# ku222/Attention-GAN

Measured on AMD Instinct MI355X. Metric: train images/sec at 256×256 stage-3, batch 24/GPU, 1/2/4/8 MI355X, higher is better.
Workload: dtype f32; 1 GPU; full 3-stage AttnGAN 64->128->256 train step: G + 3xD updates + word attention + DAMSM words/sentence loss + KL + 4x fused Adam (BASELINE.json configs[2]); workload_key=full3, batch_per_gpu=24, global_batch=24, gf_dim=32, df_dim=64, emb_dim=256, seq_len=10, text_encoder=bypassed (frozen; N(0,1) embeddings), parallelism=dp1, discriminator_streams=3, launch=eager, gradient_exchange=none (one rank), losses_finite=True

## Files before the change

### attention-gan_amd/csrc/conv_wino.hip

```cpp
#include "conv_common.h"

#include <cstring>
#include <type_traits>

using namespace agan;
using namespace agan::conv;

namespace {

typedef unsigned u32x4 __attribute__((ext_vector_type(4)));

__device__ __forceinline__ void lds_barrier_w() { asm volatile("s_waitcnt lgkmcnt(0)\n\ts_barrier" ::: "memory"); }

__global__ __launch_bounds__(256) void wino_weight_transform_kernel(const float* __restrict__ wk, float* __restrict__ U, int Kin, int Nld, int N) {
    const int total = Kin * Nld;
    for (int e = blockIdx.x * 256 + threadIdx.x; e < total; e += gridDim.x * 256) {
        const int n = e % Nld, c = e / Nld;
        float gk[3][3];
#pragma unroll
        for (int r = 0; r < 3; ++r)
#pragma unroll
            for (int s = 0; s < 3; ++s) gk[r][s] = n < N ? wk[(size_t)(c * 9 + r * 3 + s) * Nld + n] : 0.f;
        float t[4][3];
#pragma unroll
        for (int s = 0; s < 3; ++s) {
            t[0][s] = gk[0][s];
            t[1][s] = 0.5f * (gk[0][s] + gk[1][s] + gk[2][s]);
            t[2][s] = 0.5f * (gk[0][s] - gk[1][s] + gk[2][s]);
            t[3][s] = gk[2][s];
        }
        const int nch8 = Kin >> 3;
#pragma unroll
        for (int xi = 0; xi < 4; ++xi) {
            const float u0 = t[xi][0], u1 = 0.5f * (t[xi][0] + t[xi][1] + t[xi][2]), u2 = 0.5f * (t[xi][0] - t[xi][1] + t[xi][2]), u3 = t[xi][2];
            const float u[4] = {u0, u1, u2, u3};
#pragma unroll
            for (int nu = 0; nu < 4; ++nu) U[((size_t)((xi * 4 + nu) * nch8 + (c >> 3)) * Nld + n) * 8 + (c & 7)] = u[nu];
        }
    }
}

struct WinoTraits {
    int step, extra, origin;
    int cch;
    int planes, classes;
    int stages, nacc;
    int vfrags;
    int pieces;
    int ni32, ni64;
    int lds_cap;
    int s_u_second, s_raw_load, s_u_next, s_transform, s_raw_store;
    bool mulshift;
    bool store1_late;
};
constexpr WinoTraits wino_traits(WinoKind k) {
    WinoTraits t{};
    t.origin = -1; t.classes = 1; t.lds_cap = 160 * 1024; t.s_u_second = 0; t.s_raw_load = 1;
    switch (k) {
    case WinoKind::conv3x3:
        t.step = 2; t.extra = 2; t.cch = 8; t.planes = 16; t.stages = 16; t.nacc = 16; t.vfrags = 16; t.pieces = 4; t.ni32 = 7; t.ni64 = 11;
        t.s_u_next = 8; t.s_transform = 1; t.s_raw_store = 14;
        break;
    case WinoKind::conv3x3_half:
        t.step = 2; t.extra = 2; t.cch = 8; t.planes = 16; t.stages = 8; t.nacc = 8; t.vfrags = 16; t.pieces = 4; t.ni32 = 7;
        t.s_u_next = 4; t.s_transform = 1; t.s_raw_store = 6; t.lds_cap = 80 * 1024; t.mulshift = true;
        break;
    case WinoKind::conv4x4_s2:
        t.step = 4; t.extra = 2; t.cch = 8; t.planes = 36; t.stages = 36; t.nacc = 9; t.vfrags = 36; t.pieces = 4; t.ni32 = 21;
        t.s_u_next = 18; t.s_transform = 2; t.s_raw_store = 32; t.store1_late = true;
        break;
    case WinoKind::dgrad2x2_class:
        t.step = 2; t.extra = 1; t.cch = 16; t.planes = 36; t.classes = 4; t.stages = 18; t.nacc = 9; t.vfrags = 18; t.pieces = 2; t.ni32 = 11;
        t.s_u_next = 9; t.s_transform = 2; t.s_raw_store = 15; t.store1_late = true;
        break;
    }
    return t;
}

template <int D>
__device__ __forceinline__ void wino_input_f22(const float* src, int pcp, float* o, int pp) {
    float t[3][3];
#pragma unroll
    for (int j = 0; j < 3; ++j) {
        const float d0 = src[D * j], d1 = src[D * pcp + D * j], d2 = src[2 * D * pcp + D * j];
        t[0][j] = d0 - d1; t[1][j] = d1; t[2][j] = d2 - d1;
    }
#pragma unroll
    for (int xi = 0; xi < 3; ++xi) {
        o[(xi * 3 + 0) * pp] = t[xi][0] - t[xi][1]; o[(xi * 3 + 1) * pp] = t[xi][1]; o[(xi * 3 + 2) * pp] = t[xi][2] - t[xi][1];
    }
}

template <int NACC>
__device__ __forceinline__ void wino_output_2x2(const f32x16 (&acc)[NACC], int r, float (&y)[4]) {
    if constexpr (NACC == 16) {
        float c0[4], c1[4];
#pragma unroll
        for (int nu = 0; nu < 4; ++nu) {
            c0[nu] = acc[0 + nu][r] + acc[4 + nu][r] + acc[8 + nu][r];
            c1[nu] = acc[4 + nu][r] - acc[8 + nu][r] - acc[12 + nu][r];
        }
        y[0] = c0[0] + c0[1] + c0[2]; y[1] = c0[1] - c0[2] - c0[3];
        y[2] = c1[0] + c1[1] + c1[2]; y[3] = c1[1] - c1[2] - c1[3];
    } else {
        static_assert(NACC == 9, "F(2x2, 3x3) or F(2x2, 2x2)");
        float c0[3], c1[3];
#pragma unroll
        for (int nu = 0; nu < 3; ++nu) {
            c0[nu] = acc[nu][r] + acc[3 + nu][r];
            c1[nu] = acc[3 + nu][r] + acc[6 + nu][r];
        }
        y[0] = c0[0] + c0[1]; y[1] = c0[1] + c0[2];
        y[2] = c1[0] + c1[1]; y[3] = c1[1] + c1[2];
    }
}

template <WinoKind K, int NTG>
struct WinoGather {
    static constexpr WinoTraits T = wino_traits(K);
    static constexpr bool kHalf = K == WinoKind::conv3x3_half, kS2 = K == WinoKind::conv4x4_s2, kCls = K == WinoKind::dgrad2x2_class;
    static constexpr bool k3x3 = T.nacc != 9;
    static constexpr int NFW = kHalf ? 2 : 4 / NTG;
    static constexpr int NTL = 32 * NTG, LT = NTG == 1 ? 5 : 6;
    static constexpr int NI = NTG == 1 ? T.ni32 : T.ni64;
    static constexpr int CCH = T.cch, C8 = T.cch / 8;
    static constexpr int S = T.stages, SH = T.stages / 2, NACC = T.nacc;
    static constexpr int NPIECE = T.pieces * NTG;
    static constexpr int VBUF = T.vfrags * NTL * 8;
    static constexpr int STEP = T.step;
    static_assert(NI > 0, "this block size of the variant is not built: plan_wino must not route to it");
    static_assert(T.s_u_next == SH && T.s_transform + NPIECE <= S && T.s_raw_store < S, "slots of the chunk loop");

    const Geom& g;
    const WinoPlan& wp;
    int tid, lane, w, fw, tg, hh, l31, lh;
    int mt, nt, ks, py, px;
    int n0, txl, tyl, TX, TY, tx0, ty0, tb0, ihw, ohw, PR, PC, PCP, RAWBUF;
    float *raw, *V;
    __amdgpu_buffer_rsrc_t rx, rU;
    int nch8, c_beg, nch;
    int iy0, ix0;

    __device__ __forceinline__ WinoGather(const float* x, const float* U, const Geom& g_, const WinoPlan& wp_) : g(g_), wp(wp_) {
        extern __shared__ __attribute__((aligned(16))) unsigned char lds[];
        tid = threadIdx.x; lane = tid & 63;
        w = __builtin_amdgcn_readfirstlane(tid >> 6);
        fw = w % NFW; tg = kHalf ? 0 : w / NFW; hh = kHalf ? w / NFW : 0;
        l31 = lane & 31; lh = lane >> 5;
        ks = py = px = 0;
        {
            int F = xcd_contiguous(linear_block_id(), wp.mtiles * wp.ntiles * (kS2 ? wp.ksplit : T.classes));
            nt = F % wp.ntiles; F /= wp.ntiles;
            if constexpr (kS2) { mt = F % wp.mtiles; ks = F / wp.mtiles; }
            else if constexpr (kCls) { py = (F & 3) >> 1; px = F & 1; mt = F >> 2; }
            else mt = F;
        }
        n0 = nt * (NFW * 32);
        txl = wp.txl; tyl = wp.tyl;
        TX = 1 << txl; TY = 1 << tyl;
        const int bxi = mt % wp.blocks_x, byi = (mt / wp.blocks_x) % wp.blocks_y, bbi = mt / (wp.blocks_x * wp.blocks_y);
        tx0 = bxi << txl; ty0 = byi << tyl; tb0 = bbi << (LT - txl - tyl);
        ihw = g.IH * g.IW; ohw = g.OH * g.OW;
        PR = STEP * TY + T.extra; PC = STEP * TX + T.extra;
        PCP = wp.pcp;
        raw = reinterpret_cast<float*>(lds);
        RAWBUF = wp.raw_bytes >> 2;
        V = reinterpret_cast<float*>(lds + 2 * wp.raw_bytes);
        nch8 = g.Cin >> 3;
        if constexpr (kS2) { c_beg = ks * wp.chunks_per_split; nch = min(nch8, c_beg + wp.chunks_per_split) - c_beg; }
        else { c_beg = 0; nch = g.Cin >> (CCH == 8 ? 3 : 4); }
        constexpr int PPC = T.planes / T.classes;
        rx = make_rsrc(x, (size_t)g.B * g.Cin * ihw * sizeof(float));
        rU = make_rsrc(U + (size_t)(py * 2 + px) * PPC * nch8 * g.Nld * 8, (size_t)PPC * nch8 * g.Nld * 8 * sizeof(float));
        iy0 = STEP * ty0 + T.origin + py; ix0 = STEP * tx0 + T.origin + px;
    }

    __device__ __forceinline__ void stage_items(int (&it_off)[NI], unsigned (&it_lds)[NI]) const {
#pragma unroll
        for (int i = 0; i < NI; ++i) {
            const int e = tid + i * 256;
            int col, row, t2;
            if constexpr (T.mulshift) {
                const int t1 = (int)(__umul24(e, wp.mpc) >> 16);
                col = e - (int)__umul24(t1, PC);
                t2 = (int)(__umul24(t1, wp.mpr) >> 16); row = t1 - (int)__umul24(t2, PR);
            } else {
                col = e % PC; const int t1 = e / PC;
                row = t1 % PR; t2 = t1 / PR;
            }
            const int ci = t2 & (CCH - 1), b = tb0 + (t2 >> (CCH == 8 ? 3 : 4)), iy = iy0 + row, ix = ix0 + col;
            const bool ok = (e < wp.raw_items) & (b < g.B) & ((unsigned)iy < (unsigned)g.IH) & ((unsigned)ix < (unsigned)g.IW);
            if constexpr (T.mulshift) {
                it_off[i] = ok ? (int)__umul24(b * g.Cin + ci, ihw) + iy * g.IW + ix : -1;
                it_lds[i] = (unsigned)((int)__umul24(__umul24(t2, PR) + row, PCP) + col);
            } else {
                it_off[i] = ok ? (b * g.Cin + ci) * ihw + iy * g.IW + ix : -1;
                it_lds[i] = (unsigned)((t2 * PR + row) * PCP + col);
            }
        }
    }

    __device__ __forceinline__ void load_raw(const int (&it_off)[NI], int ch, float (&rv)[NI]) const {
#pragma unroll
        for (int i = 0; i < NI; ++i)
            rv[i] = buf_load_s(rx, it_off[i] >= 0 ? (unsigned)it_off[i] * 4u : kOOB, (unsigned)((c_beg + ch) * CCH * ihw) * 4u);
    }
    __device__ __forceinline__ void store_raw(const unsigned (&it_lds)[NI], int ch, const float (&rv)[NI]) const {
        float* const rb = raw + (ch & 1) * RAWBUF;
#pragma unroll
        for (int i = 0; i < NI; ++i)
            if (tid + i * 256 < wp.raw_items) rb[it_lds[i]] = rv[i];
    }
    __device__ __forceinline__ void load_u(int ch, int half, u32x4 (&uf)[SH]) const {
        const unsigned ulane = (unsigned)(min(n0 + fw * 32 + l31, g.Nld - 1) * 32 + lh * 16);
#pragma unroll
        for (int q = 0; q < SH; ++q) {
            const int s = half * SH + q;
            uf[q] = __builtin_bit_cast(u32x4, __builtin_amdgcn_raw_buffer_load_b128(
                rU, ulane, (unsigned)(((hh * S + s / C8) * nch8 + (c_beg + min(ch, nch - 1)) * C8 + s % C8) * g.Nld) * 32u, 0));
        }
    }

    __device__ __forceinline__ void transform_piece(const float* rb, float* Vb, int pi, float (&td)[NTG][4][4]) const {
        const int k = pi / T.pieces, sub = pi % T.pieces;
        const int tt = (tid >> 3) + 32 * k, ci = (tid & 7) + (kCls ? 8 * sub : 0);
        const int p = kS2 ? sub >> 1 : 0, q = kS2 ? sub & 1 : 0;
        if (!k3x3 || sub == 0) {
            const int ttx = tt & (TX - 1), tty = (tt >> txl) & (TY - 1), ttb = tt >> (txl + tyl);
            const float* const src = rb + ((ttb * CCH + ci) * PR + STEP * tty + p) * PCP + STEP * ttx + q;
            if constexpr (k3x3) {
                float d[4][4];
#pragma unroll
                for (int i = 0; i < 4; ++i) {
                    const float2 a = *reinterpret_cast<const float2*>(src + i * PCP), b = *reinterpret_cast<const float2*>(src + i * PCP + 2);
                    d[i][0] = a.x; d[i][1] = a.y; d[i][2] = b.x; d[i][3] = b.y;
                }
#pragma unroll
                for (int j = 0; j < 4; ++j) {
                    td[k][0][j] = d[0][j] - d[2][j];
                    td[k][1][j] = d[1][j] + d[2][j];
                    td[k][2][j] = d[2][j] - d[1][j];
                    td[k][3][j] = d[1][j] - d[3][j];
                }
            } else if constexpr (kS2) wino_input_f22<2>(src, PCP, Vb + (sub * 9 * NTL + tt) * 8 + ci, NTL * 8);
            else wino_input_f22<1>(src, PCP, Vb + tt * 16 + ci, NTL * 16);
        }
        if constexpr (k3x3) {
            const float (&t)[4] = td[k][sub];
            float* const o = Vb + (sub * 4 * NTL + tt) * 8 + ci;
            o[0] = t[0] - t[2]; o[NTL * 8] = t[1] + t[2]; o[2 * NTL * 8] = t[2] - t[1]; o[3 * NTL * 8] = t[1] - t[3];
        }
    }

    __device__ __forceinline__ void accumulate(f32x16 (&acc)[NACC]) const {
        int it_off[NI];
        unsigned it_lds[NI];
        stage_items(it_off, it_lds);
        float rawv[NI];
        float td[NTG][4][4];
        u32x4 ua[SH], ub[SH];
#pragma unroll
        for (int q = 0; q < NACC; ++q)
#pragma unroll
            for (int r = 0; r < 16; ++r) acc[q][r] = 0.f;
        {
            float rawv1[NI];
            load_raw(it_off, 0, rawv);
            if (!T.store1_late && nch > 1) load_raw(it_off, 1, rawv1);
            load_u(0, 0, ua);
            store_raw(it_lds, 0, rawv);
            if (nch > 1) {
                if constexpr (T.store1_late) load_raw(it_off, 1, rawv);
                else store_raw(it_lds, 1, rawv1);
            }
            lds_barrier_w();
#pragma unroll
            for (int pi = 0; pi < NPIECE; ++pi) transform_piece(raw, V, pi, td);
            if (T.store1_late && nch > 1) store_raw(it_lds, 1, rawv);
            lds_barrier_w();
        }
#pragma unroll 1
        for (int ch = 0; ch < nch; ++ch) {
            const float* Vc = V + (ch & 1) * VBUF;
            float* Vn = V + ((ch + 1) & 1) * VBUF;
            const float* rn = raw + ((ch + 1) & 1) * RAWBUF;
            const bool more = ch + 1 < nch;
            const unsigned vlane = (unsigned)(hh * S * NTL * 8 + (tg * 32 + l31) * CCH + lh * 4);
            u32x4 vf[2];
            vf[0] = *reinterpret_cast<const u32x4*>(Vc + vlane);
#pragma unroll
            for (int st = 0; st < S; ++st) {
                if (st + 1 < S) vf[(st + 1) & 1] = *reinterpret_cast<const u32x4*>(Vc + ((st + 1) / C8) * NTL * CCH + ((st + 1) % C8) * 8 + vlane);
                if (st == T.s_u_second) load_u(ch, 1, ub);
                if (st == T.s_raw_load && ch + 2 < nch) load_raw(it_off, ch + 2, rawv);
                if (st == T.s_u_next) load_u(ch + 1, 0, ua);
                if (more && st >= T.s_transform && st < T.s_transform + NPIECE) transform_piece(rn, Vn, st - T.s_transform, td);
                if (st == T.s_raw_store && ch + 2 < nch) store_raw(it_lds, ch + 2, rawv);
                const u32x4 uf = st < SH ? ua[st % SH] : ub[st % SH];
                const int a = kS2 ? st % NACC : st / C8;
#pragma unroll
                for (int j = 0; j < 4; ++j)
                    acc[a] = __builtin_amdgcn_mfma_f32_32x32x2f32(__uint_as_float(uf[j]), __uint_as_float(vf[st & 1][j]), acc[a], 0, 0, 0);
                __builtin_amdgcn_sched_barrier(0);
            }
            lds_barrier_w();
        }
    }

    __device__ __forceinline__ void epilogue(const f32x16 (&acc)[NACC], float* out) const {
        typedef float f32x2_ __attribute__((ext_vector_type(2)));
        typedef unsigned u32x2_ __attribute__((ext_vector_type(2)));
        const int lt = tg * 32 + l31;
        const int tx = lt & (TX - 1), ty = (lt >> txl) & (TY - 1), tb = lt >> (txl + tyl);
        const int b = tb0 + tb, oy = 2 * (ty0 + ty), ox = 2 * (tx0 + tx);
        const bool pvalid = (b < g.B) & (oy < (kCls ? g.OHs : g.OH)) & (ox < (kCls ? g.OWs : g.OW));
        const __amdgpu_buffer_rsrc_t ro = make_rsrc(out + (size_t)ks * wp.slab, (size_t)g.B * g.Cout * ohw * sizeof(float));
        const int nw = n0 + fw * 32;
#pragma unroll
        for (int r = 0; r < 16; ++r) {
            float y[4];
            wino_output_2x2(acc, r, y);
            const int n = nw + (r & 3) + 8 * (r >> 2) + 4 * lh;
            const bool ok = pvalid & (n < g.Cout);
            if constexpr (kCls) {
                const unsigned off = (unsigned)((b * g.Cout + n) * ohw + (2 * oy + py) * g.OW + 2 * ox + px) * 4u;
                buf_store(ro, ok ? off : kOOB, y[0]);
                buf_store(ro, ok ? off + 8u : kOOB, y[1]);
                buf_store(ro, ok ? off + (unsigned)(2 * g.OW) * 4u : kOOB, y[2]);
                buf_store(ro, ok ? off + (unsigned)(2 * g.OW + 2) * 4u : kOOB, y[3]);
            } else {
                const unsigned off = (unsigned)((b * g.Cout + n) * ohw + oy * g.OW + ox) * 4u;
                __builtin_amdgcn_raw_buffer_store_b64(__builtin_bit_cast(u32x2_, f32x2_{y[0], y[1]}), ro, ok ? off : kOOB, 0, 0);
                __builtin_amdgcn_raw_buffer_store_b64(__builtin_bit_cast(u32x2_, f32x2_{y[2], y[3]}), ro, ok ? off + (unsigned)g.OW * 4u : kOOB, 0, 0);
            }
        }
    }
};

template <int NFW>
__global__ __launch_bounds__(256, 1) void conv_wino_f32_kernel(const float* __restrict__ x, const float* __restrict__ U, float* __restrict__ out,
                                                               const Geom g, const WinoPlan wp) {
    WinoGather<WinoKind::conv3x3, 4 / NFW> k(x, U, g, wp);
    f32x16 acc[k.NACC];
    k.accumulate(acc);
    k.epilogue(acc, out);
}

__global__ __launch_bounds__(256, 2) void conv_wino_h_f32_kernel(const float* __restrict__ x, const float* __restrict__ U, float* __restrict__ out,
                                                                 const Geom g, const WinoPlan wp) {
    WinoGather<WinoKind::conv3x3_half, 1> k(x, U, g, wp);
    f32x16 acc[8];
    k.accumulate(acc);

    const int w = k.w, lane = k.lane, hh = k.hh, ohw = k.ohw;
    float* const X = k.raw;
    typedef float f32x2_ __attribute__((ext_vector_type(2)));
    typedef unsigned u32x2_ __attribute__((ext_vector_type(2)));
    const int tx = k.l31 & (k.TX - 1), ty = (k.l31 >> k.txl) & (k.TY - 1), tb = k.l31 >> (k.txl + k.tyl);
    const int b = k.tb0 + tb, oy = 2 * (k.ty0 + ty) + hh, ox = 2 * (k.tx0 + tx);
    const bool pvalid = (b < g.B) & (oy < g.OH) & (ox < g.OW);
    const __amdgpu_buffer_rsrc_t ro = make_rsrc(out, (size_t)g.B * g.Cout * ohw * sizeof(float));
    const int nw = k.n0 + k.fw * 32, pw = w ^ 2;
    const unsigned vo = pvalid ? (unsigned)((b * g.Cout + nw + 4 * k.lh) * ohw + oy * g.OW + ox) * 4u : kOOB;
    auto finish = [&](auto hc) {
        constexpr int HH = decltype(hc)::value;
        f32x2_ keep[8][2];
#pragma unroll
        for (int rp = 0; rp < 8; ++rp) {
            f32x2_ t[2][2];
#pragma unroll
            for (int x2 = 0; x2 < 2; ++x2) {
                const f32x2_ m0 = {acc[x2 * 4 + 0][2 * rp], acc[x2 * 4 + 0][2 * rp + 1]};
                const f32x2_ m1 = {acc[x2 * 4 + 1][2 * rp], acc[x2 * 4 + 1][2 * rp + 1]};
                const f32x2_ m2 = {acc[x2 * 4 + 2][2 * rp], acc[x2 * 4 + 2][2 * rp + 1]};
                const f32x2_ m3 = {acc[x2 * 4 + 3][2 * rp], acc[x2 * 4 + 3][2 * rp + 1]};
                t[x2][0] = m0 + m1 + m2;
                t[x2][1] = m1 - m2 - m3;
            }
#pragma unroll
            for (int c = 0; c < 2; ++c) {
                keep[rp][c] = t[0][c] + t[1][c];
                const f32x2_ send = HH == 0 ? t[1][c] : t[0][c];
                X[(w * 32 + (2 * rp) * 2 + c) * 64 + lane] = send[0];
                X[(w * 32 + (2 * rp + 1) * 2 + c) * 64 + lane] = send[1];
            }
        }
        lds_barrier_w();
#pragma unroll
        for (int r = 0; r < 16; ++r) {
            if (nw + 8 * (r >> 2) < g.Cout) {
                const float x0 = X[(pw * 32 + r * 2 + 0) * 64 + lane], x1 = X[(pw * 32 + r * 2 + 1) * 64 + lane];
                const float k0 = keep[r >> 1][0][r & 1], k1 = keep[r >> 1][1][r & 1];
                const f32x2_ y = HH == 0 ? f32x2_{x0 + k0, x1 + k1} : f32x2_{x0 - k0, x1 - k1};
                __builtin_amdgcn_raw_buffer_store_b64(__builtin_bit_cast(u32x2_, y), ro, vo, (unsigned)(((r & 3) + 8 * (r >> 2)) * ohw) * 4u, 0);
            }
        }
    };
    if (hh == 0) finish(std::integral_constant<int, 0>{});
    else finish(std::integral_constant<int, 1>{});
}

template <int NFW>
__global__ __launch_bounds__(256, 1) void conv_wino_s2_f32_kernel(const float* __restrict__ x, const float* __restrict__ U, float* __restrict__ out,
                                                                  const Geom g, const WinoPlan wp) {
    WinoGather<WinoKind::conv4x4_s2, 4 / NFW> k(x, U, g, wp);
    f32x16 acc[k.NACC];
    k.accumulate(acc);
    k.epilogue(acc, out);
}

template <int NFW>
__global__ __launch_bounds__(256, 1) void conv_wino_cls_f32_kernel(const float* __restrict__ x, const float* __restrict__ U, float* __restrict__ out,
                                                                   const Geom g, const WinoPlan wp) {
    WinoGather<WinoKind::dgrad2x2_class, 4 / NFW> k(x, U, g, wp);
    f32x16 acc[k.NACC];
    k.accumulate(acc);
    k.epilogue(acc, out);
}

__device__ __forceinline__ void wino_weights_f22(const float (&gk)[2][2], float* o, size_t pp) {
    const float t[3][2] = {{gk[0][0], gk[0][1]}, {gk[0][0] + gk[1][0], gk[0][1] + gk[1][1]}, {gk[1][0], gk[1][1]}};
#pragma unroll
    for (int xi = 0; xi < 3; ++xi) {
        const float u[3] = {t[xi][0], t[xi][0] + t[xi][1], t[xi][1]};
#pragma unroll
        for (int nu = 0; nu < 3; ++nu) o[(xi * 3 + nu) * pp] = u[nu];
    }
}

__global__ __launch_bounds__(256) void wino_cls_weight_transform_kernel(const float* __restrict__ wk, float* __restrict__ U, int Kin, int Nld, int N) {
    const int total = 4 * Kin * Nld, nch8 = Kin >> 3;
    for (int e = blockIdx.x * 256 + threadIdx.x; e < total; e += gridDim.x * 256) {
        const int n = e % Nld, t1 = e / Nld, c = t1 % Kin, cls = t1 / Kin;
        const float* wc = wk + (size_t)cls * Kin * 4 * Nld;
        float gk[2][2];
#pragma unroll
        for (int a = 0; a < 2; ++a)
#pragma unroll
            for (int b = 0; b < 2; ++b) gk[a][b] = n < N ? wc[(size_t)(c * 4 + (1 - a) * 2 + (1 - b)) * Nld + n] : 0.f;
        wino_weights_f22(gk, U + ((size_t)(cls * 9 * nch8 + (c >> 3)) * Nld + n) * 8 + (c & 7), (size_t)nch8 * Nld * 8);
    }
}

__global__ __launch_bounds__(256) void wino_s2_weight_transform_kernel(const float* __restrict__ wk, float* __restrict__ U, int Kin, int Nld, int N) {
    const int total = Kin * Nld, nch8 = Kin >> 3;
    for (int e = blockIdx.x * 256 + threadIdx.x; e < total; e += gridDim.x * 256) {
        const int n = e % Nld, c = e / Nld;
#pragma unroll
        for (int p = 0; p < 2; ++p)
#pragma unroll
            for (int q = 0; q < 2; ++q) {
                float gk[2][2];
#pragma unroll
                for (int a = 0; a < 2; ++a)
#pragma unroll
                    for (int b = 0; b < 2; ++b) gk[a][b] = n < N ? wk[(size_t)(c * 16 + (2 * a + p) * 4 + 2 * b + q) * Nld + n] : 0.f;
                wino_weights_f22(gk, U + ((size_t)((p * 2 + q) * 9 * nch8 + (c >> 3)) * Nld + n) * 8 + (c & 7), (size_t)nch8 * Nld * 8);
            }
    }
}

__global__ __launch_bounds__(512, 1) void conv_wino_wgrad_f32_kernel(const float* __restrict__ x, const float* __restrict__ dy, float* __restrict__ part,
                                                                     const Geom g, const WinoWgradPlan wp) {
    extern __shared__ __attribute__((aligned(16))) unsigned char lds[];
    constexpr int ZV = 16 * 64 * 8;
    float* const L = reinterpret_cast<float*>(lds);
    const int tid = threadIdx.x, lane = tid & 63;
    const int w = __builtin_amdgcn_readfirstlane(tid >> 6);
    const int up = w >> 2;
    const int fj = w & 1, fi = (w >> 1) & 1;
    const int l31 = lane & 31, lh = lane >> 5;
    int jt, it, split;
    {
        int F = xcd_contiguous(linear_block_id(), wp.jtiles * wp.itiles * wp.psplit);
        jt = F % wp.jtiles; F /= wp.jtiles;
        it = F % wp.itiles; split = F / wp.itiles;
    }
    const int j0 = jt * 64, i0 = it * 64;
    const int ihw = g.IH * g.IW;
    const int o_beg = split * wp.octs_per_split, o_end = min(wp.noct, o_beg + wp.octs_per_split);
    const __amdgpu_buffer_rsrc_t rx = make_rsrc(x, (size_t)g.B * g.Cin * ihw * sizeof(float));
    const __amdgpu_buffer_rsrc_t rd = make_rsrc(dy, (size_t)g.B * g.Cout * ihw * sizeof(float));
    const int tw8 = g.OW >> 4, th = g.OH >> 1;

    const int tj = tid & 7, tc = tid >> 3;
    float xr[16];
    float2 dr[2];
    const int xthr = (i0 + tc) * ihw + 2 * tj - 1, dthr = (j0 + tc) * ihw + 2 * tj;
    const bool cvx = i0 + tc < g.Cin, cvd = j0 + tc < g.Cout;
    const bool tj_first = tj == 0, tj_last = tj == 7;
    auto load_piece = [&](int o, int lp) {
        const bool ov = o < o_end;
        const int txo = o % tw8, t1 = o / tw8;
        const int ty = t1 % th, b = t1 / th;
        if (lp < 2) {
            const int sx = b * g.Cin * ihw + 16 * txo;
            const bool c0ok = !(tj_first & (txo == 0)), c3ok = !(tj_last & (txo == tw8 - 1));
#pragma unroll
            for (int ii = 0; ii < 2; ++ii) {
                const int i = 2 * lp + ii;
                const int iy = 2 * ty - 1 + i;
                const bool rv = cvx & (ov & ((unsigned)iy < (unsigned)g.IH));
                const unsigned ro = (unsigned)(xthr + (sx + iy * g.IW)) * 4u;
                xr[i * 4 + 0] = buf_load(rx, (rv & c0ok) ? ro : kOOB);
                const float2 mid = __builtin_bit_cast(float2, __builtin_amdgcn_raw_buffer_load_b64(rx, rv ? ro + 4u : kOOB, 0, 0));
                xr[i * 4 + 1] = mid.x;
                xr[i * 4 + 2] = mid.y;
                xr[i * 4 + 3] = buf_load(rx, (rv & c3ok) ? ro + 12u : kOOB);
            }
        } else {
            const bool dv = cvd & ov;
            const int sd = b * g.Cout * ihw + 2 * ty * g.OW + 16 * txo;
#pragma unroll
            for (int a = 0; a < 2; ++a)
                dr[a] = __builtin_bit_cast(float2, __builtin_amdgcn_raw_buffer_load_b64(rd, dv ? (unsigned)(dthr + (sd + a * g.OW)) * 4u : kOOB, 0, 0));
        }
    };
    auto load_oct = [&](int o) {
#pragma unroll
        for (int lp = 0; lp < 3; ++lp) load_piece(o, lp);
    };
    float tt_[4][4];
    auto transform_piece = [&](float* buf, int sub) {
        if (sub == 0) {
#pragma unroll
            for (int c = 0; c < 4; ++c) {
                const float d0 = xr[c], d1 = xr[4 + c], d2 = xr[8 + c], d3 = xr[12 + c];
                tt_[0][c] = d0 - d2; tt_[1][c] = d1 + d2; tt_[2][c] = d2 - d1; tt_[3][c] = d3 - d1;
            }
        }
        if (sub < 2) {
#pragma unroll
            for (int x2 = 0; x2 < 2; ++x2) {
                const int xi = 2 * sub + x2;
                const float* t = tt_[xi];
                float* o = buf + ZV + ((xi * 4) * 64 + tc) * 8 + tj;
                o[0] = t[0] - t[2]; o[64 * 8] = t[1] + t[2]; o[2 * 64 * 8] = t[2] - t[1]; o[3 * 64 * 8] = t[3] - t[1];
            }
        } else {
            const float e00 = dr[0].x, e01 = dr[0].y, e10 = dr[1].x, e11 = dr[1].y;
#pragma unroll
            for (int x2 = 0; x2 < 2; ++x2) {
                const int xi = 2 * (sub - 2) + x2;
                const float u0 = xi == 0 ? e00 : (xi == 1 ? 0.5f * (e00 + e10) : (xi == 2 ? 0.5f * (e00 - e10) : e10));
                const float u1 = xi == 0 ? e01 : (xi == 1 ? 0.5f * (e01 + e11) : (xi == 2 ? 0.5f * (e01 - e11) : e11));
                float* o = buf + ((xi * 4) * 64 + tc) * 8 + tj;
                o[0] = u0; o[64 * 8] = 0.5f * (u0 + u1); o[2 * 64 * 8] = 0.5f * (u0 - u1); o[3 * 64 * 8] = u1;
            }
        }
    };
    auto transform_store = [&](float* buf) {
#pragma unroll
        for (int tp = 0; tp < 4; ++tp) transform_piece(buf, tp);
    };

    f32x16 acc[8];
#pragma unroll
    for (int q = 0; q < 8; ++q)
#pragma unroll
        for (int r = 0; r < 16; ++r) acc[q][r] = 0.f;

    if (o_beg < o_end) {
        load_oct(o_beg);
        transform_store(L);
        load_oct(o_beg + 1);
        lds_barrier_w();
        const unsigned zl = (unsigned)(up * 8 * 64 * 8 + (fj * 32 + l31) * 8 + lh * 4), vl = (unsigned)(ZV + up * 8 * 64 * 8 + (fi * 32 + l31) * 8 + lh * 4);
        auto octet = [&](auto s0, int o) {
            constexpr int S0 = decltype(s0)::value;
            const float* cur = L + ((o - o_beg) & 1) * (2 * ZV);
            float* nxt = L + (((o - o_beg) & 1) ^ 1) * (2 * ZV);
            u32x4 zf[2], vf[2];
            zf[0] = *reinterpret_cast<const u32x4*>(cur + zl);
            vf[0] = *reinterpret_cast<const u32x4*>(cur + vl);
#pragma unroll
            for (int q = 0; q < 8; ++q) {
                if (q + 1 < 8) {
                    zf[(q + 1) & 1] = *reinterpret_cast<const u32x4*>(cur + (q + 1) * 64 * 8 + zl);
                    vf[(q + 1) & 1] = *reinterpret_cast<const u32x4*>(cur + (q + 1) * 64 * 8 + vl);
                }
                if (q >= S0 && q < S0 + 4) transform_piece(nxt, q - S0);
                if (q >= S0 + 1 && q < S0 + 4) load_piece(o + 2, q - S0 - 1);
#pragma unroll
                for (int j = 0; j < 4; ++j)
                    acc[q] = __builtin_amdgcn_mfma_f32_32x32x2f32(__uint_as_float(zf[q & 1][j]), __uint_as_float(vf[q & 1][j]), acc[q], 0, 0, 0);
#pragma unroll
                for (int j = 0; j < 4; ++j) {
                    __builtin_amdgcn_sched_group_barrier(0x008, 1, 0);
                    __builtin_amdgcn_sched_group_barrier(0x100, 1, 0);
                    __builtin_amdgcn_sched_group_barrier(0x002, 8, 0);
                    __builtin_amdgcn_sched_group_barrier(0x020, 2, 0);
                    __builtin_amdgcn_sched_group_barrier(0x200, 2, 0);
                }
                __builtin_amdgcn_sched_barrier(0);
            }
            lds_barrier_w();
        };
        if (up == 0) {
            for (int o = o_beg; o < o_end; ++o) octet(std::integral_constant<int, 0>{}, o);
        } else {
            for (int o = o_beg; o < o_end; ++o) octet(std::integral_constant<int, 4>{}, o);
        }
    }

    auto hand_over = [&](auto upc) {
        constexpr int R0 = decltype(upc)::value ? 0 : 8;
        f32x4* const mine = reinterpret_cast<f32x4*>(L) + w * (16 * 64) + lane;
#pragma unroll
        for (int q = 0; q < 8; ++q)
#pragma unroll
            for (int rq = 0; rq < 2; ++rq) {
                f32x4 v;
#pragma unroll
                for (int e = 0; e < 4; ++e) v[e] = acc[q][R0 + 4 * rq + e];
                mine[(q * 2 + rq) * 64] = v;
            }
    };
    if (up == 0) hand_over(std::integral_constant<int, 0>{});
    else hand_over(std::integral_constant<int, 1>{});
    lds_barrier_w();

    float* const o = part + (size_t)split * wp.slab;
    const __amdgpu_buffer_rsrc_t ro = make_rsrc(o, (size_t)9 * g.Cout * g.Cin * sizeof(float));
    const int ci = i0 + fi * 32 + l31;
    const int cob = j0 + fj * 32;
    const unsigned vo = ci < g.Cin ? (unsigned)(4 * lh * g.Cin + ci) * 4u : kOOB;
    const unsigned tapb = (unsigned)(g.Cout * g.Cin) * 4u;
    const f32x4* const theirs = reinterpret_cast<const f32x4*>(L) + (w ^ 4) * (16 * 64) + lane;
    auto finish = [&](auto upc) {
        constexpr int UP = decltype(upc)::value;
#pragma unroll
        for (int rq = 0; rq < 2; ++rq) {
            const int rg = 2 * UP + rq;
            if (cob + 8 * rg >= g.Cout) continue;
            f32x4 oth[8];
#pragma unroll
            for (int q = 0; q < 8; ++q) oth[q] = theirs[(q * 2 + rq) * 64];
#pragma unroll
            for (int e = 0; e < 4; ++e) {
                const int r = 4 * rg + e;
                float c[3][4];
#pragma unroll
                for (int nu = 0; nu < 4; ++nu) {
                    const float m0 = UP ? oth[nu][e] : acc[nu][r], m1 = UP ? oth[4 + nu][e] : acc[4 + nu][r];
                    const float m2 = UP ? acc[nu][r] : oth[nu][e], m3 = UP ? acc[4 + nu][r] : oth[4 + nu][e];
                    c[0][nu] = m0 + m1 + m2;
                    c[1][nu] = m1 - m2;
                    c[2][nu] = m1 + m2 + m3;
                }
                const unsigned so = (unsigned)((cob + e + 8 * rg) * g.Cin) * 4u;
#pragma unroll
                for (int rr = 0; rr < 3; ++rr) {
                    __builtin_amdgcn_raw_buffer_store_b32(__builtin_bit_cast(unsigned, c[rr][0] + c[rr][1] + c[rr][2]), ro, vo, so + (unsigned)(rr * 3 + 0) * tapb, 0);
                    __builtin_amdgcn_raw_buffer_store_b32(__builtin_bit_cast(unsigned, c[rr][1] - c[rr][2]), ro, vo, so + (unsigned)(rr * 3 + 1) * tapb, 0);
                    __builtin_amdgcn_raw_buffer_store_b32(__builtin_bit_cast(unsigned, c[rr][1] + c[rr][2] + c[rr][3]), ro, vo, so + (unsigned)(rr * 3 + 2) * tapb, 0);
                }
            }
        }
    };
    if (up == 0) finish(std::integral_constant<int, 0>{});
    else finish(std::integral_constant<int, 1>{});
}

__global__ __launch_bounds__(256) void wino_wgrad_sum_kernel(const float* __restrict__ part, int nslabs, size_t slab, int cout, int cin,
                                                             float* __restrict__ dw, int accumulate) {
    __shared__ f32x4 red[8][32];
    const int q4 = cin >> 2, n4 = 9 * cout * q4;
    const int el = threadIdx.x & 31, grp = threadIdx.x >> 5;
    for (int base = blockIdx.x * 32; base < n4; base += gridDim.x * 32) {
        const int e = base + el;
        f32x4 a = {0.f, 0.f, 0.f, 0.f};
        if (e < n4) {
            const float* src = part + (size_t)e * 4;
            int sp = grp;
            for (; sp + 24 < nslabs; sp += 32) {
                const f32x4 v0 = *reinterpret_cast<const f32x4*>(src + (size_t)sp * slab);
                const f32x4 v1 = *reinterpret_cast<const f32x4*>(src + (size_t)(sp + 8) * slab);
                const f32x4 v2 = *reinterpret_cast<const f32x4*>(src + (size_t)(sp + 16) * slab);
                const f32x4 v3 = *reinterpret_cast<const f32x4*>(src + (size_t)(sp + 24) * slab);
                a += (v0 + v1) + (v2 + v3);
            }
            for (; sp < nslabs; sp += 8) a += *reinterpret_cast<const f32x4*>(src + (size_t)sp * slab);
        }
        red[grp][el] = a;
        __syncthreads();
        if (grp == 0 && e < n4) {
#pragma unroll
            for (int k = 1; k < 8; ++k) a += red[k][el];
            const int c4 = e % q4, t1 = e / q4;
            const int co = t1 % cout, tap = t1 / cout;
            float* dst = dw + ((size_t)co * cin + 4 * c4) * 9 + tap;
#pragma unroll
            for (int k = 0; k < 4; ++k) dst[k * 9] = accumulate ? dst[k * 9] + a[k] : a[k];
        }
        __syncthreads();
    }
}

int pow2floor_log(int v) {
    int l = 0;
    while ((2 << l) <= v) ++l;
    return l;
}

}

namespace agan {
namespace conv {

WinoPlan plan_wino(const Geom& g) {
    WinoPlan p;
    memset(&p, 0, sizeof(p));
    if (g.SY == 1 && g.R == 3 && g.S == 3 && g.DY == 1 && g.OS == 1 && g.OY0 == -1 && g.IH == g.OH && g.IW == g.OW)
        p.kind = (g.Cout & 7) == 0 ? WinoKind::conv3x3_half : WinoKind::conv3x3;
    else if (g.SY == 2 && g.R == 4 && g.S == 4 && g.DY == 1 && g.OS == 1 && g.OY0 == -1 && g.IH == 2 * g.OH && g.IW == 2 * g.OW) p.kind = WinoKind::conv4x4_s2;
    else if (g.SY == 1 && g.R == 2 && g.S == 2 && g.DY == -1 && g.OS == 2 && g.OY0 == 0 && g.OY1 == 1 && g.OH == 2 * g.IH && g.OW == 2 * g.IW) p.kind = WinoKind::dgrad2x2_class;
    else return p;
    const WinoTraits T = wino_traits(p.kind);
    const bool k3x3 = p.kind == WinoKind::conv3x3 || p.kind == WinoKind::conv3x3_half;
    if ((g.OHs & 1) || (g.OWs & 1) || (g.Cin & (T.cch - 1)) || g.Cout < 32) return p;
    if (!k3x3 && g.Cout < 96) return p;
    const int tw = g.OWs / 2, th = g.OHs / 2;
    if (tw < 4) return p;
    p.nf = (g.Cout >= 96 || p.kind == WinoKind::conv3x3_half) ? 4 : 2;
    const int lt = p.nf == 4 ? 5 : 6;
    p.txl = std::min(3, pow2floor_log(tw));
    p.tyl = std::min(lt - p.txl, pow2floor_log(th));
    const int TX = 1 << p.txl, TY = 1 << p.tyl, TB = (1 << lt) >> (p.txl + p.tyl);
    p.blocks_x = cdiv(tw, TX);
    p.blocks_y = cdiv(th, TY);
    p.blocks_b = cdiv(g.B, TB);
    p.mtiles = p.blocks_x * p.blocks_y * p.blocks_b;
    p.ntiles = p.kind == WinoKind::conv3x3_half ? cdiv(g.Cout, 64) : cdiv(g.Cout, p.nf * 32);
    p.ksplit = 1;
    if (p.kind == WinoKind::conv4x4_s2 && p.mtiles * p.ntiles < 512 && p.mtiles * p.ntiles >= 256 && g.Cin >= 128) p.ksplit = 2;
    if (p.mtiles * p.ntiles * p.ksplit * T.classes < (k3x3 ? 256 : 512)) return p;
    p.chunks_per_split = cdiv(g.Cin / 8, p.ksplit);
    p.slab = ((size_t)g.B * g.Cout * g.OH * g.OW + 3) / 4 * 4;
    const int PR = T.step * TY + T.extra, PC = T.step * TX + T.extra;
    p.pcp = (PC + 1) & ~1;
    p.mpc = (65536 + PC - 1) / PC;
    p.mpr = (65536 + PR - 1) / PR;
    p.raw_items = TB * T.cch * PR * PC;
    if (p.raw_items > (lt == 5 ? T.ni32 : T.ni64) * 256) return p;
    p.raw_bytes = (TB * T.cch * PR * p.pcp * 4 + 15) & ~15;
    p.smem_bytes = 2 * p.raw_bytes + 2 * T.vfrags * (1 << lt) * 8 * 4;
    if (p.smem_bytes > T.lds_cap) return p;
    p.u_bytes = ((size_t)T.planes * (g.Cin / 8) * g.Nld * 8 * sizeof(float) + 255) / 256 * 256;
    p.ws_bytes = p.u_bytes + (p.ksplit > 1 ? p.slab * p.ksplit * sizeof(float) : 0);
    p.ok = 1;
    return p;
}

namespace {
template <auto Kernel, WinoKind K>
void launch_gather_kernel(dim3 grid, const float* in, const float* U, float* out, const Geom& g, const WinoPlan& p, hipStream_t st) {
    allow_dynamic_lds<Kernel>(wino_traits(K).lds_cap);
    AGAN_LAUNCH(Kernel, grid, dim3(256), (size_t)p.smem_bytes, st, in, U, out, g, p);
}
}

void launch_wino(const float* in, const float* wk, float* out, const Geom& g, const WinoPlan& p, void* ws, hipStream_t st) {
    float* U = static_cast<float*>(ws);
    const int total = g.Cin * g.Nld;
    const dim3 grid(p.mtiles * p.ntiles * p.ksplit * wino_traits(p.kind).classes), tgrid(std::min(cdiv(total, 256), 2048));
    switch (p.kind) {
    case WinoKind::dgrad2x2_class:
        AGAN_LAUNCH(wino_cls_weight_transform_kernel, dim3(std::min(cdiv(4 * total, 256), 4096)), dim3(256), 0, st, wk, U, g.Cin, g.Nld, g.Cout);
        launch_gather_kernel<conv_wino_cls_f32_kernel<4>, WinoKind::dgrad2x2_class>(grid, in, U, out, g, p, st);
        break;
    case WinoKind::conv4x4_s2:
        AGAN_LAUNCH(wino_s2_weight_transform_kernel, tgrid, dim3(256), 0, st, wk, U, g.Cin, g.Nld, g.Cout);
        launch_gather_kernel<conv_wino_s2_f32_kernel<4>, WinoKind::conv4x4_s2>(
            grid, in, U, p.ksplit > 1 ? reinterpret_cast<float*>(static_cast<char*>(ws) + p.u_bytes) : out, g, p, st);
        break;
    case WinoKind::conv3x3_half:
        AGAN_LAUNCH(wino_weight_transform_kernel, tgrid, dim3(256), 0, st, wk, U, g.Cin, g.Nld, g.Cout);
        launch_gather_kernel<conv_wino_h_f32_kernel, WinoKind::conv3x3_half>(grid, in, U, out, g, p, st);
        break;
    case WinoKind::conv3x3:
        AGAN_LAUNCH(wino_weight_transform_kernel, tgrid, dim3(256), 0, st, wk, U, g.Cin, g.Nld, g.Cout);
        if (p.nf == 4) launch_gather_kernel<conv_wino_f32_kernel<4>, WinoKind::conv3x3>(grid, in, U, out, g, p, st);
        else launch_gather_kernel<conv_wino_f32_kernel<2>, WinoKind::conv3x3>(grid, in, U, out, g, p, st);
        break;
    }
}

WinoWgradPlan plan_wino_wgrad(const Geom& g) {
    WinoWgradPlan p;
    memset(&p, 0, sizeof(p));
    if (!(g.SY == 1 && g.R == 3 && g.S == 3 && g.DY == 1 && g.OS == 1 && g.OY0 == -1)) return p;
    if (g.IH != g.OH || g.IW != g.OW || (g.OH & 1) || (g.OW & 15) || g.Cin < 32 || g.Cout < 32 || (g.Cin & 3) || (g.Cout & 7)) return p;
    p.noct = g.B * (g.OH / 2) * (g.OW / 16);
    p.jtiles = cdiv(g.Cout, 64);
    p.itiles = cdiv(g.Cin, 64);
    const int wgs = p.jtiles * p.itiles;
    if (p.noct < 64 * 16 || wgs > 256) return p;
    const int ps = std::max(1, std::min(256 / wgs, p.noct / 16));
    p.octs_per_split = cdiv(p.noct, ps);
    p.psplit = cdiv(p.noct, p.octs_per_split);
    p.slab = ((size_t)g.Cout * g.Cin * 9 + 3) / 4 * 4;
    p.ws_bytes = p.slab * p.psplit * sizeof(float);
    p.smem_bytes = 2 * 2 * 16 * 64 * 8 * 4;
    p.ok = 1;
    return p;
}

void launch_wino_wgrad(const float* x, const float* dy, float* part, const Geom& g, const WinoWgradPlan& p, hipStream_t st) {
    allow_dynamic_lds<conv_wino_wgrad_f32_kernel>(160 * 1024);
    AGAN_LAUNCH(conv_wino_wgrad_f32_kernel, dim3(p.jtiles * p.itiles * p.psplit), dim3(512), (size_t)p.smem_bytes, st, x, dy, part, g, p);
}

void launch_wino_wgrad_sum(const float* part, const Geom& g, const WinoWgradPlan& p, float* dw, int accumulate, hipStream_t st) {
    const int n4 = 9 * g.Cout * (g.Cin >> 2);
    AGAN_LAUNCH(wino_wgrad_sum_kernel, dim3(std::min(cdiv(n4, 32), 8192)), dim3(256), 0, st, part, p.psplit, p.slab, g.Cout, g.Cin, dw, accumulate);
}

}
}
```

Before: 1014 images/s.

## Split F(2x2) Winograd s2 and class-dgrad kernels across 512-thread wave pairs

Moves the conv4x4_s2 and dgrad2x2_class Winograd gather kernels from 256 to 512 threads per block. Each pair of waves splits the 9 Winograd accumulator planes (5 and 4), which halves per-wave accumulator registers, U fragment loads and staging items. Partial results are exchanged through LDS in a new paired epilogue before the output transform. It also adds explicit MFMA/LDS/VMEM interleaving via sched_group_barrier. The cost is an extra LDS exchange and barrier, and clamped staging indices that issue redundant loads.

```diff
diff --git a/attention-gan_amd/csrc/conv_wino.hip b/attention-gan_amd/csrc/conv_wino.hip
--- a/attention-gan_amd/csrc/conv_wino.hip
+++ b/attention-gan_amd/csrc/conv_wino.hip
@@ -44,6 +44,7 @@
     int step, extra, origin;
     int cch;
     int planes, classes;
+    int threads;
     int stages, nacc;
     int vfrags;
     int pieces;
@@ -55,7 +56,7 @@
 };
 constexpr WinoTraits wino_traits(WinoKind k) {
     WinoTraits t{};
-    t.origin = -1; t.classes = 1; t.lds_cap = 160 * 1024; t.s_u_second = 0; t.s_raw_load = 1;
+    t.origin = -1; t.classes = 1; t.lds_cap = 160 * 1024; t.s_u_second = 0; t.s_raw_load = 1; t.threads = 256;
     switch (k) {
     case WinoKind::conv3x3:
         t.step = 2; t.extra = 2; t.cch = 8; t.planes = 16; t.stages = 16; t.nacc = 16; t.vfrags = 16; t.pieces = 4; t.ni32 = 7; t.ni64 = 11;
@@ -66,12 +67,12 @@
         t.s_u_next = 4; t.s_transform = 1; t.s_raw_store = 6; t.lds_cap = 80 * 1024; t.mulshift = true;
         break;
     case WinoKind::conv4x4_s2:
-        t.step = 4; t.extra = 2; t.cch = 8; t.planes = 36; t.stages = 36; t.nacc = 9; t.vfrags = 36; t.pieces = 4; t.ni32 = 21;
-        t.s_u_next = 18; t.s_transform = 2; t.s_raw_store = 32; t.store1_late = true;
+        t.step = 4; t.extra = 2; t.cch = 8; t.planes = 36; t.threads = 512; t.stages = 20; t.nacc = 9; t.vfrags = 36; t.pieces = 4; t.ni32 = 11;
+        t.s_transform = 2; t.s_raw_store = 14; t.store1_late = true;
         break;
     case WinoKind::dgrad2x2_class:
-        t.step = 2; t.extra = 1; t.cch = 16; t.planes = 36; t.classes = 4; t.stages = 18; t.nacc = 9; t.vfrags = 18; t.pieces = 2; t.ni32 = 11;
-        t.s_u_next = 9; t.s_transform = 2; t.s_raw_store = 15; t.store1_late = true;
+        t.step = 2; t.extra = 1; t.cch = 16; t.planes = 36; t.classes = 4; t.threads = 512; t.stages = 10; t.nacc = 9; t.vfrags = 18; t.pieces = 2; t.ni32 = 6;
+        t.s_transform = 2; t.s_raw_store = 7; t.store1_late = true;
         break;
     }
     return t;
@@ -120,16 +121,19 @@
     static constexpr WinoTraits T = wino_traits(K);
     static constexpr bool kHalf = K == WinoKind::conv3x3_half, kS2 = K == WinoKind::conv4x4_s2, kCls = K == WinoKind::dgrad2x2_class;
     static constexpr bool k3x3 = T.nacc != 9;
+    static constexpr int NT = T.threads;
+    static constexpr bool kPair = NT == 512;
     static constexpr int NFW = kHalf ? 2 : 4 / NTG;
     static constexpr int NTL = 32 * NTG, LT = NTG == 1 ? 5 : 6;
     static constexpr int NI = NTG == 1 ? T.ni32 : T.ni64;
     static constexpr int CCH = T.cch, C8 = T.cch / 8;
     static constexpr int S = T.stages, SH = T.stages / 2, NACC = T.nacc;
-    static constexpr int NPIECE = T.pieces * NTG;
+    static constexpr int NPIECE = T.pieces * NTG * 256 / NT;
     static constexpr int VBUF = T.vfrags * NTL * 8;
     static constexpr int STEP = T.step;
     static_assert(NI > 0, "this block size of the variant is not built: plan_wino must not route to it");
-    static_assert(T.s_u_next == SH && T.s_transform + NPIECE <= S && T.s_raw_store < S, "slots of the chunk loop");
+    static_assert((kPair || T.s_u_next == SH) && T.s_transform + NPIECE <= S && T.s_raw_store < S, "slots of the chunk loop");
+    static_assert(!kPair || (NTG == 1 && !k3x3), "wave pairs: the F(2x2, 2x2) forms on 32-tile blocks");
 
     const Geom& g;
     const WinoPlan& wp;
@@ -145,7 +149,7 @@
         extern __shared__ __attribute__((aligned(16))) unsigned char lds[];
         tid = threadIdx.x; lane = tid & 63;
         w = __builtin_amdgcn_readfirstlane(tid >> 6);
-        fw = w % NFW; tg = kHalf ? 0 : w / NFW; hh = kHalf ? w / NFW : 0;
+        fw = w % NFW; tg = kHalf || kPair ? 0 : w / NFW; hh = kHalf || kPair ? w / NFW : 0;
         l31 = lane & 31; lh = lane >> 5;
         ks = py = px = 0;
         {
@@ -178,7 +182,7 @@
     __device__ __forceinline__ void stage_items(int (&it_off)[NI], unsigned (&it_lds)[NI]) const {
 #pragma unroll
         for (int i = 0; i < NI; ++i) {
-            const int e = tid + i * 256;
+            const int e = kPair ? min(tid + i * NT, wp.raw_items - 1) : tid + i * NT;
             int col, row, t2;
             if constexpr (T.mulshift) {
                 const int t1 = (int)(__umul24(e, wp.mpc) >> 16);
@@ -194,7 +198,7 @@
                 it_off[i] = ok ? (int)__umul24(b * g.Cin + ci, ihw) + iy * g.IW + ix : -1;
                 it_lds[i] = (unsigned)((int)__umul24(__umul24(t2, PR) + row, PCP) + col);
             } else {
-                it_off[i] = ok ? (b * g.Cin + ci) * ihw + iy * g.IW + ix : -1;
+                it_off[i] = ok ? ((b * g.Cin + ci) * ihw + iy * g.IW + ix) * (kPair ? 4 : 1) : -1;
                 it_lds[i] = (unsigned)((t2 * PR + row) * PCP + col);
             }
         }
@@ -202,14 +206,16 @@
 
     __device__ __forceinline__ void load_raw(const int (&it_off)[NI], int ch, float (&rv)[NI]) const {
 #pragma unroll
-        for (int i = 0; i < NI; ++i)
-            rv[i] = buf_load_s(rx, it_off[i] >= 0 ? (unsigned)it_off[i] * 4u : kOOB, (unsigned)((c_beg + ch) * CCH * ihw) * 4u);
+        for (int i = 0; i < NI; ++i) {
+            if constexpr (kPair) rv[i] = buf_load_s(rx, (unsigned)it_off[i], (unsigned)((c_beg + ch) * CCH * ihw) * 4u);
+            else rv[i] = buf_load_s(rx, it_off[i] >= 0 ? (unsigned)it_off[i] * 4u : kOOB, (unsigned)((c_beg + ch) * CCH * ihw) * 4u);
+        }
     }
     __device__ __forceinline__ void store_raw(const unsigned (&it_lds)[NI], int ch, const float (&rv)[NI]) const {
         float* const rb = raw + (ch & 1) * RAWBUF;
 #pragma unroll
         for (int i = 0; i < NI; ++i)
-            if (tid + i * 256 < wp.raw_items) rb[it_lds[i]] = rv[i];
+            if (kPair || tid + i * NT < wp.raw_items) rb[it_lds[i]] = rv[i];
     }
     __device__ __forceinline__ void load_u(int ch, int half, u32x4 (&uf)[SH]) const {
         const unsigned ulane = (unsigned)(min(n0 + fw * 32 + l31, g.Nld - 1) * 32 + lh * 16);
@@ -222,8 +228,8 @@
     }
 
     __device__ __forceinline__ void transform_piece(const float* rb, float* Vb, int pi, float (&td)[NTG][4][4]) const {
-        const int k = pi / T.pieces, sub = pi % T.pieces;
-        const int tt = (tid >> 3) + 32 * k, ci = (tid & 7) + (kCls ? 8 * sub : 0);
+        const int k = kPair ? 0 : pi / T.pieces, sub = kPair ? hh * NPIECE + pi : pi % T.pieces;
+        const int tt = (kPair ? (tid >> 3) & 31 : tid >> 3) + 32 * k, ci = (tid & 7) + (kCls ? 8 * sub : 0);
         const int p = kS2 ? sub >> 1 : 0, q = kS2 ? sub & 1 : 0;
         if (!k3x3 || sub == 0) {
             const int ttx = tt & (TX - 1), tty = (tt >> txl) & (TY - 1), ttb = tt >> (txl + tyl);
@@ -301,6 +307,86 @@
 #pragma unroll
                 for (int j = 0; j < 4; ++j)
                     acc[a] = __builtin_amdgcn_mfma_f32_32x32x2f32(__uint_as_float(uf[j]), __uint_as_float(vf[st & 1][j]), acc[a], 0, 0, 0);
+                __builtin_amdgcn_sched_barrier(0);
+            }
+            lds_barrier_w();
+        }
+    }
+
+    template <int HH>
+    struct Half {
+        static constexpr int P0 = HH ? 5 : 0, NP = HH ? 4 : 5;
+        static constexpr int SW = (kS2 ? 4 : 2) * NP, SWH = SW / 2;
+        static constexpr int pos(int st) { return P0 + (kS2 ? st % NP : st / 2); }
+        static constexpr int sub(int st) { return kS2 ? st / NP : st % 2; }
+    };
+    template <int HH>
+    __device__ __forceinline__ void load_u_half(int ch, int half, u32x4 (&uf)[Half<0>::SWH]) const {
+        using H = Half<HH>;
+        const unsigned ulane = (unsigned)(min(n0 + fw * 32 + l31, g.Nld - 1) * 32 + lh * 16);
+        const int c = c_beg + min(ch, nch - 1);
+#pragma unroll
+        for (int q = 0; q < H::SWH; ++q) {
+            const int st = half * H::SWH + q;
+            const int row = kS2 ? (H::sub(st) * 9 + H::pos(st)) * nch8 + c : H::pos(st) * nch8 + c * C8 + H::sub(st);
+            uf[q] = __builtin_bit_cast(u32x4, __builtin_amdgcn_raw_buffer_load_b128(rU, ulane, (unsigned)(row * g.Nld) * 32u, 0));
+        }
+    }
+    template <int HH>
+    __device__ __forceinline__ void accumulate_pair(f32x16 (&acc)[Half<0>::NP]) const {
+        using H = Half<HH>;
+        static_assert(T.s_transform + NPIECE <= Half<1>::SW && T.s_raw_store < Half<1>::SW && T.s_raw_load < T.s_raw_store, "slots of the chunk loop");
+        int it_off[NI];
+        unsigned it_lds[NI];
+        stage_items(it_off, it_lds);
+        float rawv[NI];
+        float td[NTG][4][4];
+        u32x4 ua[Half<0>::SWH], ub[Half<0>::SWH];
+#pragma unroll
+        for (int q = 0; q < H::NP; ++q)
+#pragma unroll
+            for (int r = 0; r < 16; ++r) acc[q][r] = 0.f;
+        {
+            load_raw(it_off, 0, rawv);
+            load_u_half<HH>(0, 0, ua);
+            store_raw(it_lds, 0, rawv);
+            if (nch > 1) load_raw(it_off, 1, rawv);
+            lds_barrier_w();
+#pragma unroll
+            for (int pi = 0; pi < NPIECE; ++pi) transform_piece(raw, V, pi, td);
+            if (nch > 1) store_raw(it_lds, 1, rawv);
+            lds_barrier_w();
+        }
+        const unsigned vlane = (unsigned)(l31 * CCH + lh * 4);
+        auto voff = [](int st) { return kS2 ? (H::sub(st) * 9 + H::pos(st)) * NTL * 8 : H::pos(st) * NTL * 16 + H::sub(st) * 8; };
+#pragma unroll 1
+        for (int ch = 0; ch < nch; ++ch) {
+            const float* Vc = V + (ch & 1) * VBUF + vlane;
+            float* Vn = V + ((ch + 1) & 1) * VBUF;
+            const float* rn = raw + ((ch + 1) & 1) * RAWBUF;
+            u32x4 vf[2];
+            vf[0] = *reinterpret_cast<const u32x4*>(Vc + voff(0));
+#pragma unroll
+            for (int st = 0; st < H::SW; ++st) {
+                if (st + 1 < H::SW) vf[(st + 1) & 1] = *reinterpret_cast<const u32x4*>(Vc + voff(st + 1));
+                if (st == 0) load_u_half<HH>(ch, 1, ub);
+                if (st == H::SWH) load_u_half<HH>(ch + 1, 0, ua);
+                if (st == T.s_raw_load) load_raw(it_off, min(ch + 2, nch - 1), rawv);
+                if (st >= T.s_transform && st < T.s_transform + NPIECE) transform_piece(rn, Vn, st - T.s_transform, td);
+                if (st == T.s_raw_store) store_raw(it_lds, ch + 2, rawv);
+                const u32x4 uf = st < H::SWH ? ua[st % H::SWH] : ub[st % H::SWH];
+                const int a = H::pos(st) - H::P0;
+#pragma unroll
+                for (int j = 0; j < 4; ++j)
+                    acc[a] = __builtin_amdgcn_mfma_f32_32x32x2f32(__uint_as_float(uf[j]), __uint_as_float(vf[st & 1][j]), acc[a], 0, 0, 0);
+#pragma unroll
+                for (int j = 0; j < 4; ++j) {
+                    __builtin_amdgcn_sched_group_barrier(0x008, 1, 0);
+                    __builtin_amdgcn_sched_group_barrier(0x100, 3, 0);
+                    __builtin_amdgcn_sched_group_barrier(0x002, 8, 0);
+                    __builtin_amdgcn_sched_group_barrier(0x020, 3, 0);
+                    __builtin_amdgcn_sched_group_barrier(0x200, 3, 0);
+                }
                 __builtin_amdgcn_sched_barrier(0);
             }
             lds_barrier_w();
@@ -335,6 +421,69 @@
             }
         }
     }
+
+    template <int HH>
+    __device__ __forceinline__ void epilogue_pair(const f32x16 (&acc)[Half<0>::NP], float* out) const {
+        using H = Half<HH>;
+        using O = Half<1 - HH>;
+        typedef float f32x2_ __attribute__((ext_vector_type(2)));
+        typedef unsigned u32x2_ __attribute__((ext_vector_type(2)));
+        const int tx = l31 & (TX - 1), ty = (l31 >> txl) & (TY - 1), tb = l31 >> (txl + tyl);
+        const int b = tb0 + tb, oy = 2 * (ty0 + ty), ox = 2 * (tx0 + tx);
+        const bool pvalid = (b < g.B) & (oy < (kCls ? g.OHs : g.OH)) & (ox < (kCls ? g.OWs : g.OW));
+        const __amdgpu_buffer_rsrc_t ro = make_rsrc(out + (size_t)ks * wp.slab, (size_t)g.B * g.Cout * ohw * sizeof(float));
+        const int nl = n0 + fw * 32 + 4 * lh;
+        const unsigned vp = pvalid ? (unsigned)((b * g.Cout + nl) * ohw + (kCls ? (2 * oy + py) * g.OW + 2 * ox + px : oy * g.OW + ox)) * 4u : kOOB;
+        f32x4* const X = reinterpret_cast<f32x4*>(raw);
+#pragma unroll
+        for (int q = 0; q < H::NP; ++q)
+#pragma unroll
+            for (int rq = 0; rq < 2; ++rq) {
+                f32x4 v;
+#pragma unroll
+                for (int e = 0; e < 4; ++e) v[e] = acc[q][8 * (1 - HH) + 4 * rq + e];
+                X[(w * 10 + q * 2 + rq) * 64 + lane] = v;
+            }
+        lds_barrier_w();
+#pragma unroll
+        for (int rq = 0; rq < 2; ++rq) {
+            f32x4 oth[O::NP];
+#pragma unroll
+            for (int q = 0; q < O::NP; ++q) oth[q] = X[((w ^ 4) * 10 + q * 2 + rq) * 64 + lane];
+#pragma unroll
+            for (int e = 0; e < 4; ++e) {
+                const int r = 8 * HH + 4 * rq + e;
+                float m[9];
+#pragma unroll
+                for (int p = 0; p < 9; ++p) m[p] = (p >= H::P0 && p < H::P0 + H::NP) ? acc[p - H::P0][r] : oth[p - O::P0][e];
+                float c0[3], c1[3];
+#pragma unroll
+                for (int nu = 0; nu < 3; ++nu) {
+                    c0[nu] = m[nu] + m[3 + nu];
+                    c1[nu] = m[3 + nu] + m[6 + nu];
+                }
+                const float y[4] = {c0[0] + c0[1], c0[1] + c0[2], c1[0] + c1[1], c1[1] + c1[2]};
+                const int dn = (r & 3) + 8 * (r >> 2);
+                const unsigned vo = nl + dn < g.Cout ? vp : kOOB;
+                const unsigned so = (unsigned)(dn * ohw) * 4u;
+                if constexpr (kCls) {
+                    __builtin_amdgcn_raw_buffer_store_b32(__builtin_bit_cast(unsigned, y[0]), ro, vo, so, 0);
+                    __builtin_amdgcn_raw_buffer_store_b32(__builtin_bit_cast(unsigned, y[1]), ro, vo, so + 8u, 0);
+                    __builtin_amdgcn_raw_buffer_store_b32(__builtin_bit_cast(unsigned, y[2]), ro, vo, so + (unsigned)(2 * g.OW) * 4u, 0);
+                    __builtin_amdgcn_raw_buffer_store_b32(__builtin_bit_cast(unsigned, y[3]), ro, vo, so + (unsigned)(2 * g.OW + 2) * 4u, 0);
+                } else {
+                    __builtin_amdgcn_raw_buffer_store_b64(__builtin_bit_cast(u32x2_, f32x2_{y[0], y[1]}), ro, vo, so, 0);
+                    __builtin_amdgcn_raw_buffer_store_b64(__builtin_bit_cast(u32x2_, f32x2_{y[2], y[3]}), ro, vo, so + (unsigned)g.OW * 4u, 0);
+                }
+            }
+        }
+    }
+    template <int HH>
+    __device__ __forceinline__ void run_pair(float* out) const {
+        f32x16 acc[Half<0>::NP];
+        accumulate_pair<HH>(acc);
+        epilogue_pair<HH>(acc, out);
+    }
 };
 
 template <int NFW>
@@ -401,21 +550,19 @@
 }
 
 template <int NFW>
-__global__ __launch_bounds__(256, 1) void conv_wino_s2_f32_kernel(const float* __restrict__ x, const float* __restrict__ U, float* __restrict__ out,
+__global__ __launch_bounds__(512, 1) void conv_wino_s2_f32_kernel(const float* __restrict__ x, const float* __restrict__ U, float* __restrict__ out,
                                                                   const Geom g, const WinoPlan wp) {
     WinoGather<WinoKind::conv4x4_s2, 4 / NFW> k(x, U, g, wp);
-    f32x16 acc[k.NACC];
-    k.accumulate(acc);
-    k.epilogue(acc, out);
+    if (k.hh == 0) k.template run_pair<0>(out);
+    else k.template run_pair<1>(out);
 }
 
 template <int NFW>
-__global__ __launch_bounds__(256, 1) void conv_wino_cls_f32_kernel(const float* __restrict__ x, const float* __restrict__ U, float* __restrict__ out,
+__global__ __launch_bounds__(512, 1) void conv_wino_cls_f32_kernel(const float* __restrict__ x, const float* __restrict__ U, float* __restrict__ out,
                                                                    const Geom g, const WinoPlan wp) {
     WinoGather<WinoKind::dgrad2x2_class, 4 / NFW> k(x, U, g, wp);
-    f32x16 acc[k.NACC];
-    k.accumulate(acc);
-    k.epilogue(acc, out);
+    if (k.hh == 0) k.template run_pair<0>(out);
+    else k.template run_pair<1>(out);
 }
 
 __device__ __forceinline__ void wino_weights_f22(const float (&gk)[2][2], float* o, size_t pp) {
@@ -742,9 +889,10 @@
     p.mpc = (65536 + PC - 1) / PC;
     p.mpr = (65536 + PR - 1) / PR;
     p.raw_items = TB * T.cch * PR * PC;
-    if (p.raw_items > (lt == 5 ? T.ni32 : T.ni64) * 256) return p;
+    if (p.raw_items > (lt == 5 ? T.ni32 : T.ni64) * T.threads) return p;
     p.raw_bytes = (TB * T.cch * PR * p.pcp * 4 + 15) & ~15;
     p.smem_bytes = 2 * p.raw_bytes + 2 * T.vfrags * (1 << lt) * 8 * 4;
+    if (T.threads == 512) p.smem_bytes = std::max(p.smem_bytes, 8 * 10 * 64 * 16);
     if (p.smem_bytes > T.lds_cap) return p;
     p.u_bytes = ((size_t)T.planes * (g.Cin / 8) * g.Nld * 8 * sizeof(float) + 255) / 256 * 256;
     p.ws_bytes = p.u_bytes + (p.ksplit > 1 ? p.slab * p.ksplit * sizeof(float) : 0);
@@ -756,7 +904,7 @@
 template <auto Kernel, WinoKind K>
 void launch_gather_kernel(dim3 grid, const float* in, const float* U, float* out, const Geom& g, const WinoPlan& p, hipStream_t st) {
     allow_dynamic_lds<Kernel>(wino_traits(K).lds_cap);
-    AGAN_LAUNCH(Kernel, grid, dim3(256), (size_t)p.smem_bytes, st, in, U, out, g, p);
+    AGAN_LAUNCH(Kernel, grid, dim3(wino_traits(K).threads), (size_t)p.smem_bytes, st, in, U, out, g, p);
 }
 }
 
```

Result: faster. 1029 images/s (median of 6 runs) (+1.5%).
